# sash-a/es_pytorch

Measured on AMD Instinct MI355X. Metric: env-steps/sec (whole node), Humanoid-v2 objective-ES, higher is better.
Workload: dtype bf16; 1 GPU; model=MLP(256, 256), env=Humanoid-v2, global_batch=1280, policies_per_gen=1280, episode_len=1000, seq_len=1000, objective=reward, parallelism=dp1, pair_rollout=True, eps_encoding=e4m3, noise_table_elems=250000000, n_params=166673

## Files before the change

es_pytorch_amd/ops/csrc/hip/mlp_core.h:

```cpp
#pragma once
#include "common.h"

#ifndef ES_FP8_WIDE4
#define ES_FP8_WIDE4 0
#endif

#define ES_MAXL 8
#define ES_MAXDIM 2048

#ifndef ES_HEAD_BATCH
#define ES_HEAD_BATCH 1
#endif
#define ES_HEAD_BT 8

template <int R, typename W, typename LD, typename FMA>
__device__ __forceinline__ void es_walk_drain(int r0, int st, int I, LD ld, FMA fma) {
  W w[R + 1];
  const int rl = r0 + R * st;
  const bool ok = rl < I;
#pragma unroll
  for (int u = 0; u < R; ++u) w[u] = ld(r0 + u * st);
  w[R] = ld(ok ? rl : 0);
#pragma unroll
  for (int u = 0; u < R; ++u) fma(w[u], r0 + u * st);
  if (ok) fma(w[R], rl);
}

template <typename W, typename LD, typename FMA>
__device__ __forceinline__ void es_walk_batched(int i0, int st, int I, LD ld, FMA fma) {
  const int T = (I + st - 1) / st;
  int t = 0;
  for (; t + ES_HEAD_BT <= T - 1; t += ES_HEAD_BT) {
    W w[ES_HEAD_BT];
#pragma unroll
    for (int u = 0; u < ES_HEAD_BT; ++u) w[u] = ld(i0 + (t + u) * st);
#pragma unroll
    for (int u = 0; u < ES_HEAD_BT; ++u) fma(w[u], i0 + (t + u) * st);
  }
  const int r0 = i0 + t * st;
  static_assert(ES_HEAD_BT == 8, "drain switch covers remainders 0..7");
  switch (T - 1 - t) {
    case 0: es_walk_drain<0, W>(r0, st, I, ld, fma); break;
    case 1: es_walk_drain<1, W>(r0, st, I, ld, fma); break;
    case 2: es_walk_drain<2, W>(r0, st, I, ld, fma); break;
    case 3: es_walk_drain<3, W>(r0, st, I, ld, fma); break;
    case 4: es_walk_drain<4, W>(r0, st, I, ld, fma); break;
    case 5: es_walk_drain<5, W>(r0, st, I, ld, fma); break;
    case 6: es_walk_drain<6, W>(r0, st, I, ld, fma); break;
    default: es_walk_drain<7, W>(r0, st, I, ld, fma); break;
  }
}

struct MlpShape {
  int n_layers;
  int dims[ES_MAXL + 1];
  int64_t woff[ES_MAXL];
  int64_t boff[ES_MAXL];
  int vec_ok[ES_MAXL];
  int maxdim;
};

static inline int64_t mlp_lds_bytes(int maxdim) {
  return 2 * (int64_t)maxdim * 4 + 256 * 8 * 4;
}

static inline int mlp_shape_init(MlpShape* sh, const int32_t* dims_host, int32_t ndims,
                                 int64_t row_stride) {
  if (ndims < 2 || ndims > ES_MAXL + 1) return -100;
  sh->n_layers = ndims - 1;
  int64_t off = 0;
  sh->maxdim = 0;
  for (int l = 0; l < ndims; ++l) {
    sh->dims[l] = dims_host[l];
    if (dims_host[l] > ES_MAXDIM) return -101;
    if (dims_host[l] > sh->maxdim) sh->maxdim = dims_host[l];
  }
  sh->maxdim = (sh->maxdim + 3) & ~3;
  for (int l = 0; l < sh->n_layers; ++l) {
    sh->woff[l] = off;
    off += (int64_t)sh->dims[l] * sh->dims[l + 1];
    sh->boff[l] = off;
    off += sh->dims[l + 1];
    const int O = sh->dims[l + 1];
    sh->vec_ok[l] = (O % 8 == 0) && (O <= 8 * 256) && (sh->woff[l] % 8 == 0);
  }
  if (off > row_stride) return -102;
  return 0;
}

__device__ __forceinline__ void bf8_fma(uint4 w, const float xi, float* acc) {
  const uint32_t ws[4] = {w.x, w.y, w.z, w.w};
#pragma unroll
  for (int q = 0; q < 4; ++q) {
    acc[2 * q] = fmaf(bf2f((uint16_t)(ws[q] & 0xFFFFu)), xi, acc[2 * q]);
    acc[2 * q + 1] = fmaf(bf2f((uint16_t)(ws[q] >> 16)), xi, acc[2 * q + 1]);
  }
}

__device__ __forceinline__ float* mlp_layers(const uint16_t* __restrict__ wb,
                                             const MlpShape& sh,
                                             float* bufA, float* bufB, float* partial,
                                             int tid, int nthreads, int act_final) {
  float* x = bufA;
  float* y = bufB;
  for (int l = 0; l < sh.n_layers; ++l) {
    const int I = sh.dims[l], O = sh.dims[l + 1];
    const uint16_t* Wt = wb + sh.woff[l];
    const uint16_t* Bs = wb + sh.boff[l];
    const bool do_act = (l < sh.n_layers - 1) || act_final;

    if (sh.vec_ok[l]) {
      const int OCT = O >> 3;
      const int PART = nthreads / OCT;
      const int oi = tid % OCT, ip = tid / OCT;
      float acc[8];
#pragma unroll
      for (int q = 0; q < 8; ++q) acc[q] = 0.0f;
      if (ip < PART) {
        const uint16_t* wcol = Wt + (oi << 3);
        typedef uint32_t u32x4v __attribute__((ext_vector_type(4)));
        auto ld = [&](int i) {
          u32x4v v = __builtin_nontemporal_load(
              reinterpret_cast<const u32x4v*>(wcol + (int64_t)i * O));
          uint4 w;
          w.x = v.x; w.y = v.y; w.z = v.z; w.w = v.w;
          return w;
        };
        int i = ip;
        const int step4 = PART * 4;
        if (i + 3 * PART < I) {
          uint4 c0 = ld(i), c1 = ld(i + PART), c2 = ld(i + 2 * PART), c3 = ld(i + 3 * PART);
          for (; i + 7 * PART < I; i += step4) {
            const uint4 n0 = ld(i + 4 * PART), n1 = ld(i + 5 * PART),
                        n2 = ld(i + 6 * PART), n3 = ld(i + 7 * PART);
            bf8_fma(c0, x[i], acc);
            bf8_fma(c1, x[i + PART], acc);
            bf8_fma(c2, x[i + 2 * PART], acc);
            bf8_fma(c3, x[i + 3 * PART], acc);
            c0 = n0; c1 = n1; c2 = n2; c3 = n3;
          }
          bf8_fma(c0, x[i], acc);
          bf8_fma(c1, x[i + PART], acc);
          bf8_fma(c2, x[i + 2 * PART], acc);
          bf8_fma(c3, x[i + 3 * PART], acc);
          i += step4;
        }
        for (; i < I; i += PART) bf8_fma(ld(i), x[i], acc);
#pragma unroll
        for (int q = 0; q < 8; ++q) partial[(ip * OCT + oi) * 8 + q] = acc[q];
      }
      __syncthreads();
      for (int o = tid; o < O; o += nthreads) {
        float s = bf2f(Bs[o]);
        const int oo = o >> 3, j = o & 7;
        for (int p = 0; p < PART; ++p) s += partial[(p * OCT + oo) * 8 + j];
        y[o] = do_act ? tanhf(s) : s;
      }
    } else {
      const int PART = nthreads / O;
      if (PART > 1) {
        const int oi = tid % O, ip = tid / O;
        float acc = 0.0f;
        if (ip < PART) {
#if ES_HEAD_BATCH
          es_walk_batched<uint16_t>(
              ip, PART, I, [&](int r) { return Wt[(int64_t)r * O + oi]; },
              [&](uint16_t w, int r) { acc = fmaf(bf2f(w), x[r], acc); });
#else
          int i = ip;
          const int step4 = PART * 4;
          for (; i + 3 * PART < I; i += step4) {
            const float w0 = bf2f(Wt[(int64_t)i * O + oi]);
            const float w1 = bf2f(Wt[(int64_t)(i + PART) * O + oi]);
            const float w2 = bf2f(Wt[(int64_t)(i + 2 * PART) * O + oi]);
            const float w3 = bf2f(Wt[(int64_t)(i + 3 * PART) * O + oi]);
            acc = fmaf(w0, x[i], acc);
            acc = fmaf(w1, x[i + PART], acc);
            acc = fmaf(w2, x[i + 2 * PART], acc);
            acc = fmaf(w3, x[i + 3 * PART], acc);
          }
          for (; i < I; i += PART) acc = fmaf(bf2f(Wt[(int64_t)i * O + oi]), x[i], acc);
#endif
          partial[ip * O + oi] = acc;
        }
        __syncthreads();
        for (int o = tid; o < O; o += nthreads) {
          float s = bf2f(Bs[o]);
          for (int p = 0; p < PART; ++p) s += partial[p * O + o];
          y[o] = do_act ? tanhf(s) : s;
        }
      } else {
        for (int o = tid; o < O; o += nthreads) {
          float acc = bf2f(Bs[o]);
#if ES_HEAD_BATCH
          es_walk_batched<uint16_t>(
              0, 1, I, [&](int r) { return Wt[(int64_t)r * O + o]; },
              [&](uint16_t w, int r) { acc = fmaf(bf2f(w), x[r], acc); });
#else
          int i = 0;
          for (; i + 3 < I; i += 4) {
            const float w0 = bf2f(Wt[(int64_t)i * O + o]);
            const float w1 = bf2f(Wt[(int64_t)(i + 1) * O + o]);
            const float w2 = bf2f(Wt[(int64_t)(i + 2) * O + o]);
            const float w3 = bf2f(Wt[(int64_t)(i + 3) * O + o]);
            acc = fmaf(w0, x[i], acc);
            acc = fmaf(w1, x[i + 1], acc);
            acc = fmaf(w2, x[i + 2], acc);
            acc = fmaf(w3, x[i + 3], acc);
          }
          for (; i < I; ++i) acc = fmaf(bf2f(Wt[(int64_t)i * O + o]), x[i], acc);
#endif
          y[o] = do_act ? tanhf(acc) : acc;
        }
      }
    }
    __syncthreads();
    float* t = x;
    x = y;
    y = t;
  }
  return x;
}

static inline void mlp_shape_vec_f32(MlpShape* sh, int64_t row_stride) {
  for (int l = 0; l < sh->n_layers; ++l)
    sh->vec_ok[l] = (sh->dims[l + 1] % 4 == 0) && (sh->woff[l] % 4 == 0) &&
                    (row_stride % 4 == 0);
}

__device__ __forceinline__ void f4_fma(uint4 w, const float xi, float* acc) {
  acc[0] = fmaf(__uint_as_float(w.x), xi, acc[0]);
  acc[1] = fmaf(__uint_as_float(w.y), xi, acc[1]);
  acc[2] = fmaf(__uint_as_float(w.z), xi, acc[2]);
  acc[3] = fmaf(__uint_as_float(w.w), xi, acc[3]);
}

__device__ __forceinline__ float* mlp_layers_f32(const float* __restrict__ wb,
                                                 const MlpShape& sh,
                                                 float* bufA, float* bufB, float* partial,
                                                 int tid, int nthreads, int act_final) {
  float* x = bufA;
  float* y = bufB;
  for (int l = 0; l < sh.n_layers; ++l) {
    const int I = sh.dims[l], O = sh.dims[l + 1];
    const float* Wt = wb + sh.woff[l];
    const float* Bs = wb + sh.boff[l];
    const bool do_act = (l < sh.n_layers - 1) || act_final;

    if (sh.vec_ok[l]) {
      const int QT = O >> 2;
      const bool wide = QT > nthreads;
      const int PART = wide ? 1 : nthreads / QT;
      const int ip = wide ? 0 : tid / QT;
      if (ip < PART) {
        for (int oi = wide ? tid : tid % QT; oi < QT; oi += nthreads) {
          float acc[4] = {0.0f, 0.0f, 0.0f, 0.0f};
          const float* wcol = Wt + (oi << 2);
          typedef uint32_t u32x4v __attribute__((ext_vector_type(4)));
          auto ld = [&](int i) {
            u32x4v v = __builtin_nontemporal_load(
                reinterpret_cast<const u32x4v*>(wcol + (int64_t)i * O));
            uint4 w;
            w.x = v.x; w.y = v.y; w.z = v.z; w.w = v.w;
            return w;
          };
          int i = ip;
          const int step4 = PART * 4;
          if (i + 3 * PART < I) {
            uint4 c0 = ld(i), c1 = ld(i + PART), c2 = ld(i + 2 * PART),
                  c3 = ld(i + 3 * PART);
            for (; i + 7 * PART < I; i += step4) {
              const uint4 n0 = ld(i + 4 * PART), n1 = ld(i + 5 * PART),
                          n2 = ld(i + 6 * PART), n3 = ld(i + 7 * PART);
              f4_fma(c0, x[i], acc);
              f4_fma(c1, x[i + PART], acc);
              f4_fma(c2, x[i + 2 * PART], acc);
              f4_fma(c3, x[i + 3 * PART], acc);
              c0 = n0; c1 = n1; c2 = n2; c3 = n3;
            }
            f4_fma(c0, x[i], acc);
            f4_fma(c1, x[i + PART], acc);
            f4_fma(c2, x[i + 2 * PART], acc);
            f4_fma(c3, x[i + 3 * PART], acc);
            i += step4;
          }
          for (; i < I; i += PART) f4_fma(ld(i), x[i], acc);
#pragma unroll
          for (int q = 0; q < 4; ++q) partial[ip * O + (oi << 2) + q] = acc[q];
        }
      }
      __syncthreads();
      for (int o = tid; o < O; o += nthreads) {
        float s = Bs[o];
        for (int p = 0; p < PART; ++p) s += partial[p * O + o];
        y[o] = do_act ? tanhf(s) : s;
      }
    } else {
      const int PART = nthreads / O;
      if (PART > 1) {
        const int oi = tid % O, ip = tid / O;
        float acc = 0.0f;
        if (ip < PART) {
          es_walk_batched<float>(
              ip, PART, I, [&](int r) { return Wt[(int64_t)r * O + oi]; },
              [&](float w, int r) { acc = fmaf(w, x[r], acc); });
          partial[ip * O + oi] = acc;
        }
        __syncthreads();
        for (int o = tid; o < O; o += nthreads) {
          float s = Bs[o];
          for (int p = 0; p < PART; ++p) s += partial[p * O + o];
          y[o] = do_act ? tanhf(s) : s;
        }
      } else {
        for (int o = tid; o < O; o += nthreads) {
          float acc = Bs[o];
          es_walk_batched<float>(
              0, 1, I, [&](int r) { return Wt[(int64_t)r * O + o]; },
              [&](float w, int r) { acc = fmaf(w, x[r], acc); });
          y[o] = do_act ? tanhf(acc) : acc;
        }
      }
    }
    __syncthreads();
    float* t = x;
    x = y;
    y = t;
  }
  return x;
}

struct EsTE8 { uint16_t t; uint8_t e; };
struct EsTE16 { uint16_t t; uint16_t e; };

__device__ __forceinline__ void bf8e_fma_pair(uint4 t, const float* e8, float xp,
                                              float xm, float* accp, float* accm) {
  const uint32_t ts[4] = {t.x, t.y, t.z, t.w};
#pragma unroll
  for (int q = 0; q < 4; ++q) {
    const float t0 = bf2f((uint16_t)(ts[q] & 0xFFFFu));
    const float t1 = bf2f((uint16_t)(ts[q] >> 16));
    accp[2 * q] = fmaf(t0 + e8[2 * q], xp, accp[2 * q]);
    accm[2 * q] = fmaf(t0 - e8[2 * q], xm, accm[2 * q]);
    accp[2 * q + 1] = fmaf(t1 + e8[2 * q + 1], xp, accp[2 * q + 1]);
    accm[2 * q + 1] = fmaf(t1 - e8[2 * q + 1], xm, accm[2 * q + 1]);
  }
}

__device__ __forceinline__ void mlp_layers_pair_fp8(
    const uint16_t* __restrict__ tb, const uint8_t* __restrict__ eb8,
    const MlpShape& sh, float* bufAp, float* bufAm, float* bufBp, float* bufBm,
    float* partial, int tid, int nthreads, int act_final,
    float** xp_out, float** xm_out) {
  float* xp = bufAp;
  float* xm = bufAm;
  float* yp = bufBp;
  float* ym = bufBm;
  float* partm = partial + 256 * 8;
  for (int l = 0; l < sh.n_layers; ++l) {
    const int I = sh.dims[l], O = sh.dims[l + 1];
    const uint16_t* Tt = tb + sh.woff[l];
    const uint8_t* Et8 = eb8 + sh.woff[l];
    const uint16_t* TBs = tb + sh.boff[l];
    const uint8_t* EBs8 = eb8 + sh.boff[l];
    const bool do_act = (l < sh.n_layers - 1) || act_final;

    if (sh.vec_ok[l]) {
      const int OCT = O >> 3;
      const int PART = nthreads / OCT;
      const int oi = tid % OCT, ip = tid / OCT;
      float accp[8], accm[8];
#pragma unroll
      for (int q = 0; q < 8; ++q) accp[q] = accm[q] = 0.0f;
      if (ip < PART) {
        const int ro = I & 1;
        const int I2 = (I - ro) >> 1;
        const int rs2 = 2 * O;
        const uint16_t* tcol = Tt + (oi << 3);
        const uint8_t* ecol8 = Et8 + (int64_t)ro * O + (oi << 4);
        typedef uint32_t u32x4v __attribute__((ext_vector_type(4)));
        auto lde8 = [&](int i2) {
          u32x4v v = __builtin_nontemporal_load(
              reinterpret_cast<const u32x4v*>(ecol8 + (int64_t)i2 * rs2));
          uint4 w;
          w.x = v.x; w.y = v.y; w.z = v.z; w.w = v.w;
          return w;
        };
        auto ldt = [&](int r) {
          return *reinterpret_cast<const uint4*>(tcol + (int64_t)r * O);
        };
        auto fma_pairblk = [&](const uint4& e16, const uint4& ta, const uint4& tb_,
                               int r0) {
          float e8[8];
          fp8x4_decode(e16.x, e8);
          fp8x4_decode(e16.y, e8 + 4);
          bf8e_fma_pair(ta, e8, xp[r0], xm[r0], accp, accm);
          fp8x4_decode(e16.z, e8);
          fp8x4_decode(e16.w, e8 + 4);
          bf8e_fma_pair(tb_, e8, xp[r0 + 1], xm[r0 + 1], accp, accm);
        };
        if (ro && ip == 0) {
          float e8[8];
          const uint8_t* p0 = Et8 + (oi << 3);
          fp8x4_decode(*reinterpret_cast<const uint32_t*>(p0), e8);
          fp8x4_decode(*reinterpret_cast<const uint32_t*>(p0 + 4), e8 + 4);
          bf8e_fma_pair(ldt(0), e8, xp[0], xm[0], accp, accm);
        }
        int i2 = ip;
        const int step2 = PART * 2;
#if ES_FP8_WIDE4
        const int step4w = PART * 4;
        if (i2 + 3 * PART < I2) {
          uint4 e0 = lde8(i2), e1 = lde8(i2 + PART), e2 = lde8(i2 + 2 * PART),
                e3 = lde8(i2 + 3 * PART);
          uint4 t00 = ldt(ro + 2 * i2), t01 = ldt(ro + 2 * i2 + 1);
          uint4 t10 = ldt(ro + 2 * (i2 + PART)), t11 = ldt(ro + 2 * (i2 + PART) + 1);
          uint4 t20 = ldt(ro + 2 * (i2 + 2 * PART)), t21 = ldt(ro + 2 * (i2 + 2 * PART) + 1);
          uint4 t30 = ldt(ro + 2 * (i2 + 3 * PART)), t31 = ldt(ro + 2 * (i2 + 3 * PART) + 1);
          for (; i2 + 7 * PART < I2; i2 += step4w) {
            const uint4 ne0 = lde8(i2 + 4 * PART), ne1 = lde8(i2 + 5 * PART),
                        ne2 = lde8(i2 + 6 * PART), ne3 = lde8(i2 + 7 * PART);
            const uint4 nt00 = ldt(ro + 2 * (i2 + 4 * PART)),
                        nt01 = ldt(ro + 2 * (i2 + 4 * PART) + 1),
                        nt10 = ldt(ro + 2 * (i2 + 5 * PART)),
                        nt11 = ldt(ro + 2 * (i2 + 5 * PART) + 1),
                        nt20 = ldt(ro + 2 * (i2 + 6 * PART)),
                        nt21 = ldt(ro + 2 * (i2 + 6 * PART) + 1),
                        nt30 = ldt(ro + 2 * (i2 + 7 * PART)),
                        nt31 = ldt(ro + 2 * (i2 + 7 * PART) + 1);
            fma_pairblk(e0, t00, t01, ro + 2 * i2);
            fma_pairblk(e1, t10, t11, ro + 2 * (i2 + PART));
            fma_pairblk(e2, t20, t21, ro + 2 * (i2 + 2 * PART));
            fma_pairblk(e3, t30, t31, ro + 2 * (i2 + 3 * PART));
            e0 = ne0; e1 = ne1; e2 = ne2; e3 = ne3;
            t00 = nt00; t01 = nt01; t10 = nt10; t11 = nt11;
            t20 = nt20; t21 = nt21; t30 = nt30; t31 = nt31;
          }
          fma_pairblk(e0, t00, t01, ro + 2 * i2);
          fma_pairblk(e1, t10, t11, ro + 2 * (i2 + PART));
          fma_pairblk(e2, t20, t21, ro + 2 * (i2 + 2 * PART));
          fma_pairblk(e3, t30, t31, ro + 2 * (i2 + 3 * PART));
          i2 += step4w;
        }
#else
        if (i2 + PART < I2) {
          uint4 e0 = lde8(i2), e1 = lde8(i2 + PART);
          uint4 t00 = ldt(ro + 2 * i2), t01 = ldt(ro + 2 * i2 + 1);
          uint4 t10 = ldt(ro + 2 * (i2 + PART)), t11 = ldt(ro + 2 * (i2 + PART) + 1);
          for (; i2 + 3 * PART < I2; i2 += step2) {
            const uint4 ne0 = lde8(i2 + 2 * PART), ne1 = lde8(i2 + 3 * PART);
            const uint4 nt00 = ldt(ro + 2 * (i2 + 2 * PART)),
                        nt01 = ldt(ro + 2 * (i2 + 2 * PART) + 1),
                        nt10 = ldt(ro + 2 * (i2 + 3 * PART)),
                        nt11 = ldt(ro + 2 * (i2 + 3 * PART) + 1);
            fma_pairblk(e0, t00, t01, ro + 2 * i2);
            fma_pairblk(e1, t10, t11, ro + 2 * (i2 + PART));
            e0 = ne0; e1 = ne1;
            t00 = nt00; t01 = nt01; t10 = nt10; t11 = nt11;
          }
          fma_pairblk(e0, t00, t01, ro + 2 * i2);
          fma_pairblk(e1, t10, t11, ro + 2 * (i2 + PART));
          i2 += step2;
        }
#endif
        for (; i2 < I2; i2 += PART)
          fma_pairblk(lde8(i2), ldt(ro + 2 * i2), ldt(ro + 2 * i2 + 1), ro + 2 * i2);
#pragma unroll
        for (int q = 0; q < 8; ++q) {
          partial[(ip * OCT + oi) * 8 + q] = accp[q];
          partm[(ip * OCT + oi) * 8 + q] = accm[q];
        }
      }
      __syncthreads();
      for (int o = tid; o < O; o += nthreads) {
        const float tB = bf2f(TBs[o]), eB = fp8_byte(EBs8[o]);
        float sp = tB + eB, sm = tB - eB;
        const int oo = o >> 3, j = o & 7;
        for (int p = 0; p < PART; ++p) {
          sp += partial[(p * OCT + oo) * 8 + j];
          sm += partm[(p * OCT + oo) * 8 + j];
        }
        yp[o] = do_act ? tanhf(sp) : sp;
        ym[o] = do_act ? tanhf(sm) : sm;
      }
    } else {
      const int PART = nthreads / O;
      if (PART > 1) {
        const int oi = tid % O, ip = tid / O;
        float accp = 0.0f, accm = 0.0f;
        if (ip < PART) {
#if ES_HEAD_BATCH
          es_walk_batched<EsTE8>(
              ip, PART, I,
              [&](int r) {
                return EsTE8{Tt[(int64_t)r * O + oi], Et8[(int64_t)r * O + oi]};
              },
              [&](EsTE8 w, int r) {
                const float tw = bf2f(w.t), ew = fp8_byte(w.e);
                accp = fmaf(tw + ew, xp[r], accp);
                accm = fmaf(tw - ew, xm[r], accm);
              });
#else
          for (int i = ip; i < I; i += PART) {
            const float tw = bf2f(Tt[(int64_t)i * O + oi]);
            const float ew = fp8_byte(Et8[(int64_t)i * O + oi]);
            accp = fmaf(tw + ew, xp[i], accp);
            accm = fmaf(tw - ew, xm[i], accm);
          }
#endif
          partial[ip * O + oi] = accp;
          partm[ip * O + oi] = accm;
        }
        __syncthreads();
        for (int o = tid; o < O; o += nthreads) {
          const float tB = bf2f(TBs[o]), eB = fp8_byte(EBs8[o]);
          float sp = tB + eB, sm = tB - eB;
          for (int p = 0; p < PART; ++p) {
            sp += partial[p * O + o];
            sm += partm[p * O + o];
          }
          yp[o] = do_act ? tanhf(sp) : sp;
          ym[o] = do_act ? tanhf(sm) : sm;
        }
      } else {
        for (int o = tid; o < O; o += nthreads) {
          const float tB = bf2f(TBs[o]), eB = fp8_byte(EBs8[o]);
          float accp = tB + eB, accm = tB - eB;
#if ES_HEAD_BATCH
          es_walk_batched<EsTE8>(
              0, 1, I,
              [&](int r) {
                return EsTE8{Tt[(int64_t)r * O + o], Et8[(int64_t)r * O + o]};
              },
              [&](EsTE8 w, int r) {
                const float tw = bf2f(w.t), ew = fp8_byte(w.e);
                accp = fmaf(tw + ew, xp[r], accp);
                accm = fmaf(tw - ew, xm[r], accm);
              });
#else
          for (int i = 0; i < I; ++i) {
            const float tw = bf2f(Tt[(int64_t)i * O + o]);
            const float ew = fp8_byte(Et8[(int64_t)i * O + o]);
            accp = fmaf(tw + ew, xp[i], accp);
            accm = fmaf(tw - ew, xm[i], accm);
          }
#endif
          yp[o] = do_act ? tanhf(accp) : accp;
          ym[o] = do_act ? tanhf(accm) : accm;
        }
      }
    }
    __syncthreads();
    float* t = xp; xp = yp; yp = t;
    t = xm; xm = ym; ym = t;
  }
  *xp_out = xp;
  *xm_out = xm;
}

__device__ __forceinline__ float es_actnoise(uint64_t seed, uint64_t ctr) {
  esrng::f32x4 v = esrng::normal4(ctr, seed, 0xACu);
  return v.x;
}
// ... 177 lines not shown
```

es_pytorch_amd/ops/csrc/hip/rollout_loco.hip:

```cpp
#include "mlp_core.h"

#ifndef ES_DYN_DEPTH8
#define ES_DYN_DEPTH8 1
#endif

struct LocoArgs {
  int S;
  int A;
  int D;
  int goal;
  int terminate;
  int noiseless_from;
  int bins;
  int act_mode;
  int eps;
  int wrow0;
  float leak, ctrl, alive_bonus, fall_thr, dt, ob_clip;
  int64_t row_stride;
};

struct LocoPtrs {
  const uint16_t* weights;
  const float *obmean, *obstd, *ac_std_dev;
  const uint64_t* seed_dev;
// ... 413 lines not shown
}

__global__ void __launch_bounds__(256)
loco_episode_kernel(MlpShape sh, LocoArgs la, LocoPtrs P, int member_base, int n_steps,
                    int salt_base) {
  ES_LOCO_CARVE();
  const int b = member_base + blockIdx.x;
  for (int t = 1; t <= n_steps; ++t)
    loco_step_body(sh, la, P, b, (uint64_t)(salt_base + t), bufA, bufB, partial, raws,
                   abuf, sc);
}

__global__ void __launch_bounds__(512)
loco_episode512_kernel(MlpShape sh, LocoArgs la, LocoPtrs P, int member_base,
                       int n_steps, int salt_base) {
  extern __shared__ __attribute__((aligned(16))) char smem[];
  float* bufA = reinterpret_cast<float*>(smem);
  float* bufB = bufA + sh.maxdim;
  float* partial = bufB + sh.maxdim;
  float* raws = partial + 512 * 8;
  float* abuf = raws + ((la.S + 3) & ~3);
  float* sc = abuf + 64;
  const int b = member_base + blockIdx.x;
  for (int t = 1; t <= n_steps; ++t)
    loco_step_body(sh, la, P, b, (uint64_t)(salt_base + t), bufA, bufB, partial, raws,
                   abuf, sc);
}

__global__ void __launch_bounds__(256)
loco_step_f32_kernel(MlpShape sh, LocoArgs la, LocoPtrs P, uint64_t salt) {
  ES_LOCO_CARVE();
  loco_step_body<float>(sh, la, P, blockIdx.x, salt, bufA, bufB, partial, raws, abuf, sc);
}

__global__ void __launch_bounds__(256)
loco_episode_f32_kernel(MlpShape sh, LocoArgs la, LocoPtrs P, int member_base,
                        int n_steps, int salt_base) {
  ES_LOCO_CARVE();
  const int b = member_base + blockIdx.x;
  for (int t = 1; t <= n_steps; ++t)
    loco_step_body<float>(sh, la, P, b, (uint64_t)(salt_base + t), bufA, bufB, partial,
                          raws, abuf, sc);
}

__global__ void __launch_bounds__(512)
loco_episode512_f32_kernel(MlpShape sh, LocoArgs la, LocoPtrs P, int member_base,
                           int n_steps, int salt_base) {
  extern __shared__ __attribute__((aligned(16))) char smem[];
  float* bufA = reinterpret_cast<float*>(smem);
  float* bufB = bufA + sh.maxdim;
  float* partial = bufB + sh.maxdim;
  float* raws = partial + 512 * 8;
  float* abuf = raws + ((la.S + 3) & ~3);
  float* sc = abuf + 64;
  const int b = member_base + blockIdx.x;
  for (int t = 1; t <= n_steps; ++t)
    loco_step_body<float>(sh, la, P, b, (uint64_t)(salt_base + t), bufA, bufB, partial,
                          raws, abuf, sc);
}

__global__ void __launch_bounds__(256)
loco_fwd_kernel(MlpShape sh, LocoArgs la, LocoPtrs P, uint64_t salt, float* act_glob) {
  ES_LOCO_CARVE();
  (void)sc;
  const int b = blockIdx.x;
  loco_fwd_body(sh, la, P, b, salt, bufA, bufB, partial, raws, abuf);
  if (threadIdx.x < la.A) act_glob[(int64_t)b * 64 + threadIdx.x] = abuf[threadIdx.x];
}

template <int G>
__global__ void __launch_bounds__(256)
loco_dyn_kernel(LocoArgs la, LocoPtrs P, const float* act_glob, int n_pop) {
  extern __shared__ __attribute__((aligned(16))) char smem[];
  const int S = la.S;
  const int Spad = (S + 3) & ~3;
  float* raws = reinterpret_cast<float*>(smem);
  float* abuf = raws + G * Spad;
  float* partial = abuf + G * 64;
  const int tid = threadIdx.x, nth = blockDim.x;
  const int b0 = blockIdx.x * G;
  const int gs = min(G, n_pop - b0);

#pragma unroll
  for (int g = 0; g < G; ++g) {
    const float* sb = P.s_glob + (int64_t)(b0 + g) * S;
    for (int i = tid; i < S; i += nth) raws[g * Spad + i] = g < gs ? sb[i] : 0.0f;
    if (tid < la.A)
      abuf[g * 64 + tid] = g < gs ? act_glob[(int64_t)(b0 + g) * 64 + tid] : 0.0f;
  }
  __syncthreads();

  const int OCT = S >> 3;
  const int PART = nth / OCT;
  const int oi = tid % OCT, ip = tid / OCT;
  if (ip < PART) {
    float acc[G][8];
#pragma unroll
    for (int g = 0; g < G; ++g)
#pragma unroll
      for (int q = 0; q < 8; ++q) acc[g][q] = 0.0f;
    const uint16_t* acol = P.Am + (oi << 3);
    auto ld = [&](int i) {
      return *reinterpret_cast<const uint4*>(acol + (int64_t)i * S);
    };
    auto fmaG = [&](const uint4& c, int i) {
#pragma unroll
      for (int g = 0; g < G; ++g) bf8_fma(c, raws[g * Spad + i], acc[g]);
    };
    int i = ip;
    const int step4 = PART * 4;
    if (i + 3 * PART < S) {
      uint4 c0 = ld(i), c1 = ld(i + PART), c2 = ld(i + 2 * PART), c3 = ld(i + 3 * PART);
      for (; i + 7 * PART < S; i += step4) {
        const uint4 n0 = ld(i + 4 * PART), n1 = ld(i + 5 * PART),
                    n2 = ld(i + 6 * PART), n3 = ld(i + 7 * PART);
        fmaG(c0, i);
        fmaG(c1, i + PART);
        fmaG(c2, i + 2 * PART);
        fmaG(c3, i + 3 * PART);
        c0 = n0; c1 = n1; c2 = n2; c3 = n3;
      }
      fmaG(c0, i);
      fmaG(c1, i + PART);
      fmaG(c2, i + 2 * PART);
      fmaG(c3, i + 3 * PART);
      i += step4;
    }
    for (; i < S; i += PART) fmaG(ld(i), i);
#pragma unroll
    for (int g = 0; g < G; ++g)
#pragma unroll
      for (int q = 0; q < 8; ++q)
        partial[g * 2048 + (ip * OCT + oi) * 8 + q] = acc[g][q];
  }
  __syncthreads();

  for (int g = 0; g < gs; ++g)
    loco_dyn_finish(la, P, b0 + g, raws + g * Spad, abuf + g * 64,
                    partial + g * 2048, tid, nth);
}

template <int G>
static int loco_launch_dyn(const LocoArgs& la, const LocoPtrs& P, const float* act_glob,
                           int n_pop, hipStream_t stream) {
  const int Spad = (la.S + 3) & ~3;
  const unsigned lds = (unsigned)((G * Spad + G * 64 + G * 2048) * sizeof(float));
  const unsigned grid = (unsigned)((n_pop + G - 1) / G);
  loco_dyn_kernel<G><<<dim3(grid), dim3(256), lds, stream>>>(la, P, act_glob, n_pop);
  ES_CHECK_LAUNCH();
  return 0;
}


__device__ __forceinline__ void loco_dyn_partials_pair(
    const uint16_t* Am, int S, const float* rawsP, const float* rawsM,
    float* partP, float* partM, int tid, int nth) {
  const int OCT = S >> 3;
  const int PART = nth / OCT;
  const int oi = tid % OCT, ip = tid / OCT;
  float accp[8], accm[8];
#pragma unroll
  for (int q = 0; q < 8; ++q) accp[q] = accm[q] = 0.0f;
  if (ip < PART) {
    const uint16_t* acol = Am + (oi << 3);
    auto ld = [&](int i) {
      return *reinterpret_cast<const uint4*>(acol + (int64_t)i * S);
    };
    auto fma2 = [&](const uint4& c, int i) {
      bf8_fma(c, rawsP[i], accp);
      bf8_fma(c, rawsM[i], accm);
    };
    int i = ip;
    const int step4 = PART * 4;
#if ES_DYN_DEPTH8
    if (i + 7 * PART < S) {
      uint4 c0 = ld(i), c1 = ld(i + PART), c2 = ld(i + 2 * PART), c3 = ld(i + 3 * PART);
      uint4 d0 = ld(i + 4 * PART), d1 = ld(i + 5 * PART), d2 = ld(i + 6 * PART),
            d3 = ld(i + 7 * PART);
      for (; i + 11 * PART < S; i += step4) {
        const uint4 n0 = ld(i + 8 * PART), n1 = ld(i + 9 * PART),
                    n2 = ld(i + 10 * PART), n3 = ld(i + 11 * PART);
        fma2(c0, i);
        fma2(c1, i + PART);
        fma2(c2, i + 2 * PART);
        fma2(c3, i + 3 * PART);
        c0 = d0; c1 = d1; c2 = d2; c3 = d3;
        d0 = n0; d1 = n1; d2 = n2; d3 = n3;
      }
      if (i < S) fma2(c0, i);
      if (i + PART < S) fma2(c1, i + PART);
      if (i + 2 * PART < S) fma2(c2, i + 2 * PART);
      if (i + 3 * PART < S) fma2(c3, i + 3 * PART);
      if (i + 4 * PART < S) fma2(d0, i + 4 * PART);
      if (i + 5 * PART < S) fma2(d1, i + 5 * PART);
      if (i + 6 * PART < S) fma2(d2, i + 6 * PART);
      if (i + 7 * PART < S) fma2(d3, i + 7 * PART);
      i += 8 * PART;
    }
#else
    if (i + 3 * PART < S) {
      uint4 c0 = ld(i), c1 = ld(i + PART), c2 = ld(i + 2 * PART), c3 = ld(i + 3 * PART);
      for (; i + 7 * PART < S; i += step4) {
        const uint4 n0 = ld(i + 4 * PART), n1 = ld(i + 5 * PART),
                    n2 = ld(i + 6 * PART), n3 = ld(i + 7 * PART);
        fma2(c0, i);
        fma2(c1, i + PART);
        fma2(c2, i + 2 * PART);
        fma2(c3, i + 3 * PART);
        c0 = n0; c1 = n1; c2 = n2; c3 = n3;
      }
      fma2(c0, i);
      fma2(c1, i + PART);
      fma2(c2, i + 2 * PART);
      fma2(c3, i + 3 * PART);
      i += step4;
    }
#endif
    for (; i < S; i += PART) fma2(ld(i), i);
#pragma unroll
    for (int q = 0; q < 8; ++q) {
      partP[(ip * OCT + oi) * 8 + q] = accp[q];
      partM[(ip * OCT + oi) * 8 + q] = accm[q];
    }
  }
  __syncthreads();
}

#ifndef ES_DYN_EARLY
#define ES_DYN_EARLY 0
#endif

template <typename EB>
__device__ __forceinline__ void loco_pair_step_body(
    const MlpShape& sh, const LocoArgs& la, const LocoPtrs& P,
    const uint16_t* tb, const EB* eb, int bp, int bm, uint64_t salt,
    float* bufAp, float* bufAm, float* bufBp, float* bufBm, float* partial,
    float* rawsP, float* rawsM, float* abufP, float* abufM,
    float* partA = nullptr) {
  const int tid = threadIdx.x, nth = blockDim.x;
  loco_build_obs_pair(la, P, bp, bm, bufAp, bufAm, rawsP, rawsM, tid, nth);
  __syncthreads();
  const bool early = ES_DYN_EARLY && partA != nullptr && la.S % 8 == 0;
  if (early)
    loco_dyn_partials_pair(P.Am, la.S, rawsP, rawsM, partA, partA + 2048,
                           tid, nth);
  float *ap, *am;
  if constexpr (sizeof(EB) == 1)
    mlp_layers_pair_fp8(tb, (const uint8_t*)eb, sh, bufAp, bufAm, bufBp, bufBm,
                        partial, tid, nth, 1, &ap, &am);
  else
    mlp_layers_pair(tb, (const uint16_t*)eb, sh, bufAp, bufAm, bufBp, bufBm,
                    partial, tid, nth, 1, &ap, &am);
  loco_decode_action(sh, la, P, bp, salt, ap, abufP, tid);
  loco_decode_action(sh, la, P, bm, salt, am, abufM, tid);
  __syncthreads();
  float* pd = early ? partA : partial;
  if (!early && la.S % 8 == 0)
    loco_dyn_partials_pair(P.Am, la.S, rawsP, rawsM, partial, partial + 2048,
                           tid, nth);
  loco_dyn_finish_pair(la, P, bp, bm, rawsP, rawsM, abufP, abufM, pd, pd + 2048, tid,
                       nth);
}

#define ES_LOCO_PAIR_CARVE()                                     \
  extern __shared__ __attribute__((aligned(16))) char smem[];    \
  float* bufAp = reinterpret_cast<float*>(smem);                 \
  float* bufAm = bufAp + sh.maxdim;                              \
  float* bufBp = bufAm + sh.maxdim;                              \
  float* bufBm = bufBp + sh.maxdim;                              \
  float* partial = bufBm + sh.maxdim;             \
  float* rawsP = partial + 2 * 256 * 8;                          \
  float* rawsM = rawsP + ((la.S + 3) & ~3);                      \
  float* abufP = rawsM + ((la.S + 3) & ~3);                      \
  float* abufM = abufP + 64;                                     \
  float* partA = ES_DYN_EARLY ? abufM + 64 : nullptr;            \
  const int q = blockIdx.x;                                      \
  const int p = q / la.eps, e = q % la.eps;                      \
  const int bp = p * la.eps + e;                                 \
  const int bm = (n_pairs + p) * la.eps + e;                     \
  const auto* ebp = eb + (int64_t)p * la.row_stride;

#ifndef ES_PAIR_MINWAVES
#define ES_PAIR_MINWAVES 1
#endif
__global__ void __launch_bounds__(256, ES_PAIR_MINWAVES)
loco_pair_step_kernel(MlpShape sh, LocoArgs la, LocoPtrs P, const uint16_t* tb,
                      const uint16_t* eb, int n_pairs, uint64_t salt) {
  ES_LOCO_PAIR_CARVE();
  loco_pair_step_body(sh, la, P, tb, ebp, bp, bm, salt, bufAp, bufAm, bufBp, bufBm,
                      partial, rawsP, rawsM, abufP, abufM, partA);
}

__global__ void __launch_bounds__(256, ES_PAIR_MINWAVES)
loco_pair_step_fp8_kernel(MlpShape sh, LocoArgs la, LocoPtrs P, const uint16_t* tb,
                          const uint8_t* eb, int n_pairs, uint64_t salt) {
  ES_LOCO_PAIR_CARVE();
  loco_pair_step_body(sh, la, P, tb, ebp, bp, bm, salt, bufAp, bufAm, bufBp, bufBm,
                      partial, rawsP, rawsM, abufP, abufM, partA);
}

__global__ void __launch_bounds__(256, 4)
loco_pair_episode_kernel(MlpShape sh, LocoArgs la, LocoPtrs P, const uint16_t* tb,
                         const uint16_t* eb, int n_pairs, int n_steps,
                         int salt_base) {
  ES_LOCO_PAIR_CARVE();
#pragma clang loop unroll(disable)
  for (int t = 1; t <= n_steps; ++t)
    loco_pair_step_body(sh, la, P, tb, ebp, bp, bm, (uint64_t)(salt_base + t),
                        bufAp, bufAm, bufBp, bufBm, partial, rawsP, rawsM, abufP,
                        abufM, partA);
}


static int loco_prepare(MlpShape* sh, LocoArgs* la, const int32_t* dims_host, int32_t ndims,
                        int64_t row_stride, float ob_clip, int32_t sdim, int32_t adim,
                        int32_t goal_flag, int32_t terminate, int32_t noiseless_from,
                        int32_t bins, int32_t eps, int32_t act_mode, float leak,
                        float ctrl, float alive_bonus, float fall_thr, float dt,
                        unsigned* lds) {
  int rc = mlp_shape_init(sh, dims_host, ndims, row_stride);
  if (rc) return rc;
  if (adim > 64 || sdim > ES_MAXDIM) return -103;
  if (sh->dims[0] != sdim + (goal_flag ? 2 : 0)) return -104;
  int out_dim = adim;
  if (bins > 1) out_dim = adim * bins;
  else if (act_mode == 2) out_dim = adim + 1;
  else if (act_mode == 3) out_dim = adim * 2;
  if (sh->dims[sh->n_layers] != out_dim) return -105;
  la->S = sdim; la->A = adim; la->D = sh->dims[0]; la->goal = goal_flag;
  la->terminate = terminate; la->noiseless_from = noiseless_from; la->bins = bins;
  la->act_mode = act_mode;
  la->eps = eps > 0 ? eps : 1;
  la->wrow0 = 0;
  la->leak = leak; la->ctrl = ctrl; la->alive_bonus = alive_bonus; la->fall_thr = fall_thr;
  la->dt = dt; la->ob_clip = ob_clip; la->row_stride = row_stride;
  *lds = (unsigned)(mlp_lds_bytes(sh->maxdim) + (((sdim + 3) & ~3) + 64 + 8) * 4);
  return 0;
}

static LocoPtrs loco_ptrs(const void* weights, const void* obmean, const void* obstd,
                          const void* ac_std_dev, const void* seed_dev, void* s_glob,
                          void* pos, const void* goal, const void* Am, const void* Bm,
                          const void* b0, const void* wv, const void* wa, const void* wy,
                          const void* wh, void* alive, void* rew_total, void* member_steps,
                          void* behv, void* mo_sum, void* mo_sumsq) {
  LocoPtrs P;
  P.weights = (const uint16_t*)weights;
  P.obmean = (const float*)obmean; P.obstd = (const float*)obstd;
  P.ac_std_dev = (const float*)ac_std_dev; P.seed_dev = (const uint64_t*)seed_dev;
  P.s_glob = (float*)s_glob; P.pos = (float*)pos; P.goal = (const float*)goal;
  P.Am = (const uint16_t*)Am; P.Bm = (const float*)Bm; P.b0 = (const float*)b0;
  P.wv = (const float*)wv; P.wa = (const float*)wa; P.wy = (const float*)wy;
  P.wh = (const float*)wh; P.alive = (float*)alive; P.rew_total = (float*)rew_total;
  P.member_steps = (float*)member_steps; P.behv = (float*)behv;
  P.mo_sum = (float*)mo_sum; P.mo_sumsq = (float*)mo_sumsq;
  return P;
}

extern "C" int es_loco_step(const void* weights, const void* obmean, const void* obstd,
                            const int32_t* dims_host, int32_t ndims, const void* seed_dev,
                            uint64_t salt, float ob_clip, const void* ac_std_dev,
                            int64_t row_stride,
                            void* s_glob, void* pos, const void* goal, const void* Am,
                            const void* Bm, const void* b0, const void* wv, const void* wa,
                            const void* wy, const void* wh, void* alive, void* rew_total,
                            void* member_steps, void* behv, void* mo_sum, void* mo_sumsq,
                            int32_t n_pop, int32_t sdim, int32_t adim, int32_t goal_flag,
                            int32_t terminate, int32_t noiseless_from, int32_t bins,
                            int32_t eps, int32_t act_mode, float leak, float ctrl,
                            float alive_bonus, float fall_thr, float dt, void* stream) {
  MlpShape sh;
  LocoArgs la;
  unsigned lds;
  int rc = loco_prepare(&sh, &la, dims_host, ndims, row_stride, ob_clip, sdim, adim,
                        goal_flag, terminate, noiseless_from, bins, eps, act_mode, leak,
                        ctrl, alive_bonus, fall_thr, dt, &lds);
  if (rc) return rc;
  LocoPtrs P = loco_ptrs(weights, obmean, obstd, ac_std_dev, seed_dev, s_glob, pos, goal,
                         Am, Bm, b0, wv, wa, wy, wh, alive, rew_total, member_steps, behv,
                         mo_sum, mo_sumsq);
  loco_step_kernel<<<dim3((unsigned)n_pop), dim3(256), lds, (hipStream_t)stream>>>(
      sh, la, P, salt);
  ES_CHECK_LAUNCH();
  return 0;
}

extern "C" int es_loco_step_split(
    const void* weights, const void* obmean, const void* obstd,
    const int32_t* dims_host, int32_t ndims, const void* seed_dev, uint64_t salt,
    float ob_clip, const void* ac_std_dev, int64_t row_stride, void* s_glob, void* pos,
    const void* goal, const void* Am, const void* Bm, const void* b0, const void* wv,
    const void* wa, const void* wy, const void* wh, void* alive, void* rew_total,
    void* member_steps, void* behv, void* mo_sum, void* mo_sumsq, int32_t n_pop,
    int32_t sdim, int32_t adim, int32_t goal_flag, int32_t terminate,
    int32_t noiseless_from, int32_t bins, int32_t eps, int32_t act_mode, float leak,
    float ctrl, float alive_bonus, float fall_thr, float dt, void* act_glob, int32_t G,
    void* stream) {
  MlpShape sh;
  LocoArgs la;
  unsigned lds;
  int rc = loco_prepare(&sh, &la, dims_host, ndims, row_stride, ob_clip, sdim, adim,
                        goal_flag, terminate, noiseless_from, bins, eps, act_mode, leak,
                        ctrl, alive_bonus, fall_thr, dt, &lds);
  if (rc) return rc;
  if (sdim % 8 != 0) return -106;
  LocoPtrs P = loco_ptrs(weights, obmean, obstd, ac_std_dev, seed_dev, s_glob, pos, goal,
                         Am, Bm, b0, wv, wa, wy, wh, alive, rew_total, member_steps, behv,
                         mo_sum, mo_sumsq);
  hipStream_t s = (hipStream_t)stream;
  loco_fwd_kernel<<<dim3((unsigned)n_pop), dim3(256), lds, s>>>(sh, la, P, salt,
                                                                (float*)act_glob);
  ES_CHECK_LAUNCH();
  switch (G) {
    case 2: return loco_launch_dyn<2>(la, P, (const float*)act_glob, n_pop, s);
    case 4: return loco_launch_dyn<4>(la, P, (const float*)act_glob, n_pop, s);
    case 5: return loco_launch_dyn<5>(la, P, (const float*)act_glob, n_pop, s);
    case 8: return loco_launch_dyn<8>(la, P, (const float*)act_glob, n_pop, s);
    default: return -107;
  }
}

extern "C" int es_loco_pair_step(
    const void* theta_row, const void* eps_rows, const void* obmean,
    const void* obstd, const int32_t* dims_host, int32_t ndims, const void* seed_dev,
    uint64_t salt, float ob_clip, const void* ac_std_dev, int64_t row_stride,
    void* s_glob, void* pos, const void* goal, const void* Am, const void* Bm,
    const void* b0, const void* wv, const void* wa, const void* wy, const void* wh,
    void* alive, void* rew_total, void* member_steps, void* behv, void* mo_sum,
    void* mo_sumsq, int32_t n_pairs, int32_t sdim, int32_t adim, int32_t goal_flag,
    int32_t terminate, int32_t noiseless_from, int32_t bins, int32_t eps,
    int32_t act_mode, float leak, float ctrl, float alive_bonus, float fall_thr,
    float dt, void* stream) {
  MlpShape sh;
  LocoArgs la;
  unsigned lds_unused;
  int rc = loco_prepare(&sh, &la, dims_host, ndims, row_stride, ob_clip, sdim, adim,
                        goal_flag, terminate, noiseless_from, bins, eps, act_mode, leak,
                        ctrl, alive_bonus, fall_thr, dt, &lds_unused);
  if (rc) return rc;
  LocoPtrs P = loco_ptrs(nullptr, obmean, obstd, ac_std_dev, seed_dev, s_glob, pos,
                         goal, Am, Bm, b0, wv, wa, wy, wh, alive, rew_total,
                         member_steps, behv, mo_sum, mo_sumsq);
  const int Spad = (sdim + 3) & ~3;
  const unsigned lds =
      (unsigned)((4 * sh.maxdim + 2 * 256 * 8 + 2 * Spad + 2 * 64 +
                  (ES_DYN_EARLY ? 2 * 2048 : 0)) * sizeof(float));
  const unsigned grid = (unsigned)(n_pairs * la.eps);
  loco_pair_step_kernel<<<dim3(grid), dim3(256), lds, (hipStream_t)stream>>>(
      sh, la, P, (const uint16_t*)theta_row, (const uint16_t*)eps_rows, n_pairs, salt);
  ES_CHECK_LAUNCH();
  return 0;
}

extern "C" int es_loco_pair_step_fp8(
    const void* theta_row, const void* eps_rows, const void* obmean,
    const void* obstd, const int32_t* dims_host, int32_t ndims, const void* seed_dev,
    uint64_t salt, float ob_clip, const void* ac_std_dev, int64_t row_stride,
    void* s_glob, void* pos, const void* goal, const void* Am, const void* Bm,
    const void* b0, const void* wv, const void* wa, const void* wy, const void* wh,
    void* alive, void* rew_total, void* member_steps, void* behv, void* mo_sum,
    void* mo_sumsq, int32_t n_pairs, int32_t sdim, int32_t adim, int32_t goal_flag,
// ... 161 lines not shown
```

Measured before the change: 21.56 million env-steps/s.

## Software-pipeline fp8 pair MLP and dynamics partials with row streams and packed FMA

Replaces the fp8 pair-rollout inner loop and the dynamics matrix partials loop with explicitly double/triple-buffered load sets separated by scheduling barriers, so global loads for the next block are in flight while the current block is consumed. Adds a row-stream address helper, nontemporal loads for the noise stream, hardware packed fp8-to-f32 conversion, and packed 2-wide FMA on bf16 weights. The episode kernel keeps the old path via a template flag. Risks higher register pressure from the extra buffered sets, which could reduce occupancy.

Result: faster. 22.22 million env-steps/s (median of 6 runs) (+3.1%).

```diff
diff --git a/es_pytorch_amd/ops/csrc/hip/mlp_core.h b/es_pytorch_amd/ops/csrc/hip/mlp_core.h
--- a/es_pytorch_amd/ops/csrc/hip/mlp_core.h
+++ b/es_pytorch_amd/ops/csrc/hip/mlp_core.h
@@ -12,6 +12,50 @@
 #define ES_HEAD_BATCH 1
 #endif
 #define ES_HEAD_BT 8
+
+#ifndef ES_STREAM_PIPE
+#define ES_STREAM_PIPE 1
+#endif
+#ifndef ES_STREAM_SADDR
+#define ES_STREAM_SADDR 0
+#endif
+
+typedef uint32_t es_u32x4 __attribute__((ext_vector_type(4)));
+
+struct EsRowStream {
+#if ES_STREAM_SADDR
+  const char* ub;
+  uint32_t lane;
+  uint32_t sb;
+  __device__ __forceinline__ EsRowStream(const void* base, int row0, int rstep,
+                                         int rbytes, int lane_bytes)
+      : ub(reinterpret_cast<const char*>(base)),
+        lane((uint32_t)(row0 * rbytes + lane_bytes)),
+        sb((uint32_t)(rstep * rbytes)) {}
+  __device__ __forceinline__ const char* at(int k) const {
+    return ub + (size_t)(uint32_t)(lane + (uint32_t)k * sb);
+  }
+  __device__ __forceinline__ void advance(int k) { lane += (uint32_t)k * sb; }
+#else
+  const char* lb;
+  int row, rstep;
+  int64_t rbytes;
+  __device__ __forceinline__ EsRowStream(const void* base, int row0, int rstep_,
+                                         int rbytes_, int lane_bytes)
+      : lb(reinterpret_cast<const char*>(base) + lane_bytes),
+        row(row0), rstep(rstep_), rbytes(rbytes_) {}
+  __device__ __forceinline__ const char* at(int k) const {
+    return lb + (int64_t)(row + k * rstep) * rbytes;
+  }
+  __device__ __forceinline__ void advance(int k) { row += k * rstep; }
+#endif
+  __device__ __forceinline__ es_u32x4 ld(int k) const {
+    return *reinterpret_cast<const es_u32x4*>(at(k));
+  }
+  __device__ __forceinline__ es_u32x4 ld_nt(int k) const {
+    return __builtin_nontemporal_load(reinterpret_cast<const es_u32x4*>(at(k)));
+  }
+};
 
 template <int R, typename W, typename LD, typename FMA>
 __device__ __forceinline__ void es_walk_drain(int r0, int st, int I, LD ld, FMA fma) {
@@ -94,6 +138,23 @@
   for (int q = 0; q < 4; ++q) {
     acc[2 * q] = fmaf(bf2f((uint16_t)(ws[q] & 0xFFFFu)), xi, acc[2 * q]);
     acc[2 * q + 1] = fmaf(bf2f((uint16_t)(ws[q] >> 16)), xi, acc[2 * q + 1]);
+  }
+}
+
+__device__ __forceinline__ uint4 es_as_uint4(es_u32x4 v) {
+  uint4 w;
+  w.x = v.x; w.y = v.y; w.z = v.z; w.w = v.w;
+  return w;
+}
+
+__device__ __forceinline__ void bf8_fma_pk(es_u32x4 w, float xi, es_f32x2* acc2) {
+  const uint32_t ws[4] = {w.x, w.y, w.z, w.w};
+  const es_f32x2 x2 = {xi, xi};
+#pragma unroll
+  for (int q = 0; q < 4; ++q) {
+    const es_f32x2 w2 = {__builtin_bit_cast(float, ws[q] << 16),
+                         __builtin_bit_cast(float, ws[q] & 0xFFFF0000u)};
+    acc2[q] = __builtin_elementwise_fma(w2, x2, acc2[q]);
   }
 }
 
@@ -347,6 +408,24 @@
   }
 }
 
+__device__ __forceinline__ void bf8e_fma_pair_pk(es_u32x4 t, uint32_t elo, uint32_t ehi,
+                                                 float xp, float xm, es_f32x2* ap,
+                                                 es_f32x2* am) {
+  const uint32_t ts[4] = {t.x, t.y, t.z, t.w};
+  const es_f32x2 e2[4] = {__builtin_amdgcn_cvt_pk_f32_fp8(elo, false),
+                          __builtin_amdgcn_cvt_pk_f32_fp8(elo, true),
+                          __builtin_amdgcn_cvt_pk_f32_fp8(ehi, false),
+                          __builtin_amdgcn_cvt_pk_f32_fp8(ehi, true)};
+  const es_f32x2 xp2 = {xp, xp}, xm2 = {xm, xm};
+#pragma unroll
+  for (int q = 0; q < 4; ++q) {
+    const es_f32x2 t2 = {__builtin_bit_cast(float, ts[q] << 16),
+                         __builtin_bit_cast(float, ts[q] & 0xFFFF0000u)};
+    ap[q] = __builtin_elementwise_fma(t2 + e2[q], xp2, ap[q]);
+    am[q] = __builtin_elementwise_fma(t2 - e2[q], xm2, am[q]);
+  }
+}
+
 __device__ __forceinline__ void mlp_layers_pair_fp8(
     const uint16_t* __restrict__ tb, const uint8_t* __restrict__ eb8,
     const MlpShape& sh, float* bufAp, float* bufAm, float* bufBp, float* bufBm,
@@ -408,7 +487,80 @@
         }
         int i2 = ip;
         const int step2 = PART * 2;
-#if ES_FP8_WIDE4
+#if ES_STREAM_PIPE
+        const int nmin = I2 / PART;
+        if (nmin >= 2) {
+          const int T = (nmin - 2) >> 2;
+          const int rem = (I2 - 1 - ip) / PART + 1 - 4 * T - 2;
+          EsRowStream es(Et8 + (int64_t)ro * O, ip, PART, 2 * O, oi << 4);
+          EsRowStream ta(Tt + (int64_t)ro * O, ip, PART, 4 * O, oi << 4);
+          EsRowStream tb(Tt + (int64_t)(ro + 1) * O, ip, PART, 4 * O, oi << 4);
+          const float* xqp = xp + ro + 2 * ip;
+          const float* xqm = xm + ro + 2 * ip;
+          es_f32x2 a2p[4], a2m[4];
+#pragma unroll
+          for (int q = 0; q < 4; ++q) {
+            a2p[q] = es_f32x2{accp[2 * q], accp[2 * q + 1]};
+            a2m[q] = es_f32x2{accm[2 * q], accm[2 * q + 1]};
+          }
+          struct Slot { es_u32x4 e, a, b; };
+          auto ldslot = [&](Slot& s, int k) {
+            s.e = es.ld_nt(k);
+            s.a = ta.ld(k);
+            s.b = tb.ld(k);
+          };
+          auto eatslot = [&](const Slot& s, int k) {
+            const float* qp = xqp + 2 * k * PART;
+            const float* qm = xqm + 2 * k * PART;
+            bf8e_fma_pair_pk(s.a, s.e.x, s.e.y, qp[0], qm[0], a2p, a2m);
+            bf8e_fma_pair_pk(s.b, s.e.z, s.e.w, qp[1], qm[1], a2p, a2m);
+          };
+          struct Set { Slot s[2]; };
+          auto fill = [&](Set& w) {
+            ldslot(w.s[0], 0);
+            ldslot(w.s[1], 1);
+            es.advance(2);
+            ta.advance(2);
+            tb.advance(2);
+          };
+          auto eat = [&](const Set& w) {
+            eatslot(w.s[0], 0);
+            eatslot(w.s[1], 1);
+            xqp += 4 * PART;
+            xqm += 4 * PART;
+          };
+          Set c, n;
+          fill(c);
+          for (int t = T; t > 0; --t) {
+            fill(n); eat(c);
+            __builtin_amdgcn_sched_barrier(0);
+            fill(c); eat(n);
+            __builtin_amdgcn_sched_barrier(0);
+          }
+          Slot f[4];
+#pragma unroll
+          for (int k = 0; k < 4; ++k) f[k].e = f[k].a = f[k].b = es_u32x4{0u, 0u, 0u, 0u};
+#pragma unroll
+          for (int k = 0; k < 2; ++k)
+            if (k < rem) ldslot(f[k], k);
+          __builtin_amdgcn_sched_barrier(0);
+          eat(c);
+#pragma unroll
+          for (int k = 0; k < 4; ++k) {
+            __builtin_amdgcn_sched_barrier(0);
+            if (k + 2 < 4 && k + 2 < rem) ldslot(f[k + 2], k + 2);
+            __builtin_amdgcn_sched_barrier(0);
+            if (k < rem) eatslot(f[k], k);
+          }
+#pragma unroll
+          for (int q = 0; q < 4; ++q) {
+            accp[2 * q] = a2p[q].x; accp[2 * q + 1] = a2p[q].y;
+            accm[2 * q] = a2m[q].x; accm[2 * q + 1] = a2m[q].y;
+          }
+          i2 = I2;
+        }
+        (void)step2;
+#elif ES_FP8_WIDE4
         const int step4w = PART * 4;
         if (i2 + 3 * PART < I2) {
           uint4 e0 = lde8(i2), e1 = lde8(i2 + PART), e2 = lde8(i2 + 2 * PART),
diff --git a/es_pytorch_amd/ops/csrc/hip/rollout_loco.hip b/es_pytorch_amd/ops/csrc/hip/rollout_loco.hip
--- a/es_pytorch_amd/ops/csrc/hip/rollout_loco.hip
+++ b/es_pytorch_amd/ops/csrc/hip/rollout_loco.hip
@@ -589,6 +589,7 @@
 }
 
 
+template <bool PIPE = true>
 __device__ __forceinline__ void loco_dyn_partials_pair(
     const uint16_t* Am, int S, const float* rawsP, const float* rawsM,
     float* partP, float* partM, int tid, int nth) {
@@ -609,6 +610,69 @@
     };
     int i = ip;
     const int step4 = PART * 4;
+    constexpr bool kPipe = PIPE && ES_STREAM_PIPE;
+    if constexpr (kPipe) {
+    const int nmin = S / PART;
+    if (nmin >= 8) {
+      const int T = (nmin - 8) / 12;
+      const int rem = (S - 1 - ip) / PART + 1 - 12 * T - 8;
+      EsRowStream as(Am, ip, PART, 2 * S, oi << 4);
+      const float* xP = rawsP + ip;
+      const float* xM = rawsM + ip;
+      es_f32x2 a2p[4], a2m[4];
+#pragma unroll
+      for (int q = 0; q < 4; ++q) a2p[q] = a2m[q] = es_f32x2{0.0f, 0.0f};
+      struct Set { es_u32x4 v[4]; };
+      auto fill = [&](Set& s) {
+#pragma unroll
+        for (int k = 0; k < 4; ++k) s.v[k] = as.ld(k);
+        as.advance(4);
+      };
+      auto eat = [&](const Set& s) {
+#pragma unroll
+        for (int k = 0; k < 4; ++k) {
+          bf8_fma_pk(s.v[k], xP[k * PART], a2p);
+          bf8_fma_pk(s.v[k], xM[k * PART], a2m);
+        }
+        xP += 4 * PART;
+        xM += 4 * PART;
+      };
+      Set c, d, n;
+      fill(c);
+      fill(d);
+      for (int t = T; t > 0; --t) {
+        fill(n); eat(c);
+        __builtin_amdgcn_sched_barrier(0);
+        fill(c); eat(d);
+        __builtin_amdgcn_sched_barrier(0);
+        fill(d); eat(n);
+        __builtin_amdgcn_sched_barrier(0);
+      }
+      es_u32x4 f[12];
+#pragma unroll
+      for (int k = 0; k < 12; ++k)
+        if (k < rem) f[k] = as.ld(k);
+      __builtin_amdgcn_sched_barrier(0);
+      eat(c);
+      __builtin_amdgcn_sched_barrier(0);
+      eat(d);
+      __builtin_amdgcn_sched_barrier(0);
+#pragma unroll
+      for (int k = 0; k < 12; ++k) {
+        if (k < rem) {
+          bf8_fma_pk(f[k], xP[k * PART], a2p);
+          bf8_fma_pk(f[k], xM[k * PART], a2m);
+        }
+      }
+#pragma unroll
+      for (int q = 0; q < 4; ++q) {
+        accp[2 * q] = a2p[q].x; accp[2 * q + 1] = a2p[q].y;
+        accm[2 * q] = a2m[q].x; accm[2 * q + 1] = a2m[q].y;
+      }
+      i = S;
+    }
+    }
+    if constexpr (!kPipe) {
 #if ES_DYN_DEPTH8
     if (i + 7 * PART < S) {
       uint4 c0 = ld(i), c1 = ld(i + PART), c2 = ld(i + 2 * PART), c3 = ld(i + 3 * PART);
@@ -653,6 +717,7 @@
       i += step4;
     }
 #endif
+    }
     for (; i < S; i += PART) fma2(ld(i), i);
 #pragma unroll
     for (int q = 0; q < 8; ++q) {
@@ -667,7 +732,7 @@
 #define ES_DYN_EARLY 0
 #endif
 
-template <typename EB>
+template <typename EB, bool PIPE = true>
 __device__ __forceinline__ void loco_pair_step_body(
     const MlpShape& sh, const LocoArgs& la, const LocoPtrs& P,
     const uint16_t* tb, const EB* eb, int bp, int bm, uint64_t salt,
@@ -679,7 +744,7 @@
   __syncthreads();
   const bool early = ES_DYN_EARLY && partA != nullptr && la.S % 8 == 0;
   if (early)
-    loco_dyn_partials_pair(P.Am, la.S, rawsP, rawsM, partA, partA + 2048,
+    loco_dyn_partials_pair<PIPE>(P.Am, la.S, rawsP, rawsM, partA, partA + 2048,
                            tid, nth);
   float *ap, *am;
   if constexpr (sizeof(EB) == 1)
@@ -693,7 +758,7 @@
   __syncthreads();
   float* pd = early ? partA : partial;
   if (!early && la.S % 8 == 0)
-    loco_dyn_partials_pair(P.Am, la.S, rawsP, rawsM, partial, partial + 2048,
+    loco_dyn_partials_pair<PIPE>(P.Am, la.S, rawsP, rawsM, partial, partial + 2048,
                            tid, nth);
   loco_dyn_finish_pair(la, P, bp, bm, rawsP, rawsM, abufP, abufM, pd, pd + 2048, tid,
                        nth);
@@ -743,7 +808,7 @@
   ES_LOCO_PAIR_CARVE();
 #pragma clang loop unroll(disable)
   for (int t = 1; t <= n_steps; ++t)
-    loco_pair_step_body(sh, la, P, tb, ebp, bp, bm, (uint64_t)(salt_base + t),
+    loco_pair_step_body<uint16_t, false>(sh, la, P, tb, ebp, bp, bm, (uint64_t)(salt_base + t),
                         bufAp, bufAm, bufBp, bufBm, partial, rawsP, rawsM, abufP,
                         abufM, partA);
 }
```
